# statgen/demuxlet

Measured on AMD Instinct MI355X. Metric: cell-SNP-sample triples/sec (singlet+doublet llk); HBM GB/s vs roofline, higher is better.
Workload: dtype f64

## Files before the change

demuxlet_amd/csrc/dmx_engine.hip:

```cpp
#include <hip/hip_runtime.h>

#include <algorithm>
#include <chrono>
#include <cmath>
#include <mutex>
#include <cstdlib>
#include <cstring>
#include <condition_variable>
#include <deque>
#include <new>
#include <memory>
#include <functional>
#include <thread>
#include <type_traits>
#include <unordered_map>
#include <cxxabi.h>
#include <string>
#include <numeric>
#include <vector>

#include "dmx_internal.hpp"
extern char** environ;
#include "dmx_log.hpp"
#include "dmx_engine_state.hpp"
// ... 3553 lines not shown
#pragma unroll
        for (int i = 0; i < 9; ++i) { P0[i] = P[i]; P1[i] = P[9 + i]; }
        const g_t* gr = &s_g[ti * GS];
        const double a0 = (double)gr[j * 3], a1 = (double)gr[j * 3 + 1], a2 = (double)gr[j * 3 + 2];
        const double aj[3] = {a0, a1, a2};
#pragma unroll
        for (int kk = 0; kk < NK; ++kk) {
          const int k = min(kb * NK + kk, V - 1);
          const double b0 = (double)gr[k * 3], b1 = (double)gr[k * 3 + 1], b2 = (double)gr[k * 3 + 2];
          const double bk[3] = {b0, b1, b2};
          double s0 = (aj[0] * bk[0]) * P0[0], s1 = (aj[0] * bk[0]) * P1[0];
#pragma unroll
          for (int l = 0; l < 3; ++l)
#pragma unroll
            for (int m = 0; m < 3; ++m) {
              if (l == 0 && m == 0) continue;
              const double gp = aj[l] * bk[m];
              s0 += (gp * P0[l * 3 + m]);
              s1 += (gp * P1[l * 3 + m]);
            }
          if (CHK) ok &= __builtin_amdgcn_class(s0, 0x100) && __builtin_amdgcn_class(s1, 0x100);
          acc[kk][0] += dmx_log2_fast_pinned(s0, s_log, lk);
          acc[kk][1] += dmx_log2_fast_pinned(s1, s_log, lk);
        }
      }
    }
    DMX_K2_SYNC();
  }
  if (cell_ok) {
    if constexpr (SYMU) {
#pragma unroll
      for (int su = 0; su < 2; ++su) {
        const int u = tid + TPC * su, d = 1 + (u >> kUSh);
        if (d < kUV / 2 || (d == kUV / 2 && uj[su] < kUV / 2)) {
          double* o = grid + (((size_t)cell * V + uj[su]) * V + uk[su]) * A;
          o[0] = acc[2 * su][0]; o[1] = acc[2 * su][1];
          double* o2 = grid + (((size_t)cell * V + uk[su]) * V + uj[su]) * A;
          o2[0] = acc[2 * su + 1][0]; o2[1] = acc[2 * su + 1][1];
        }
      }
    } else
    if (owner) {
#pragma unroll
      for (int kk = 0; kk < NK; ++kk) {
        const int k = kb * NK + kk;
        if (k < V) {
          double* o = grid + (((size_t)cell * V + j) * V + k) * A;
          o[0] = acc[kk][0]; o[1] = acc[kk][1];
        }
      }
    }
    if (tid < 2 && blockIdx.y == 0) l00[(size_t)cell * A + tid] = acc00;
    if (!ok) flag_cell(flagged, cell);
  }
#undef DMX_K2_SYNC
}
template <int TPC, int NK, int MINW = 1, bool GD = false, bool CHK = true, int TP = 32>
__global__ __launch_bounds__(kThreads, (MINW == 1 && TPC == 64) ? 3 : MINW) void k_doublet_a2(PileupView pv, int nrd_width, const float* __restrict__ g,
                                                         const double* __restrict__ gp0, const double* __restrict__ tabs,
                                                         const double* __restrict__ alpha,
                                                         const int32_t* __restrict__ sched, int32_t V, int32_t GS,
                                                         double* __restrict__ grid, double* __restrict__ l00,
                                                         uint8_t* __restrict__ flagged, const double* __restrict__ pfin, const double* __restrict__ pseed) {
  a2_body<TPC, NK, MINW, GD, CHK, TP, false>(pv, nrd_width, g, gp0, tabs, alpha, sched, V, GS, grid, l00, flagged, pfin, pseed);
}
template <int MINW>
__global__ __launch_bounds__(kThreads, MINW) void k_doublet_a2u(PileupView pv, int nrd_width, const float* __restrict__ g,
                                                          const double* __restrict__ gp0, const double* __restrict__ tabs,
                                                          const double* __restrict__ alpha,
                                                          const int32_t* __restrict__ sched, int32_t V, int32_t GS,
                                                          double* __restrict__ grid, double* __restrict__ l00,
                                                          uint8_t* __restrict__ flagged, const double* __restrict__ pfin, const double* __restrict__ pseed) {
  a2_body<256, 4, MINW, true, false, 32, true>(pv, nrd_width, g, gp0, tabs, alpha, sched, V, GS, grid, l00, flagged, pfin, pseed);
}
__global__ __launch_bounds__(kThreads, 3) void k_doublet_a2u16(PileupView pv, int nrd_width, const float* __restrict__ g,
                                                          const double* __restrict__ gp0, const double* __restrict__ tabs,
                                                          const double* __restrict__ alpha,
                                                          const int32_t* __restrict__ sched, int32_t V, int32_t GS,
                                                          double* __restrict__ grid, double* __restrict__ l00,
                                                          uint8_t* __restrict__ flagged, const double* __restrict__ pfin, const double* __restrict__ pseed) {
  a2_body<64, 4, 1, false, false, 32, true>(pv, nrd_width, g, gp0, tabs, alpha, sched, V, GS, grid, l00, flagged, pfin, pseed);
}

template <int TPC, int NK>
__global__ __launch_bounds__(kThreads, 3) void k_doublet_a2f(PileupView pv, int nrd_width, const float* __restrict__ g,
                                                         const double* __restrict__ gp0, const double* __restrict__ tabs,
                                                         const double* __restrict__ alpha,
                                                         const int32_t* __restrict__ sched, int32_t V, int32_t GS,
                                                         double* __restrict__ grid, double* __restrict__ l00,
                                                         uint8_t* __restrict__ flagged) {
  constexpr int A = 2, TP = 32;
  constexpr int CPW = kThreads / TPC;
  constexpr int T00 = TP + 2;
#define DMX_K2_SYNC() do { if (TPC == 64) { DMX_WAVE_LDS_ORDER(); } else { __syncthreads(); } } while (0)
  extern __shared__ __attribute__((aligned(16))) unsigned char s_raw[];
  __shared__ double s_tab[kTab2];
  const double* s_log = s_tab + kLut2;
  const int t = threadIdx.x;
  stage_k2_tables(s_tab, tabs, t, kThreads);
  __syncthreads();

  const int cw = t / TPC, tid = t % TPC;
  constexpr bool SHARE = TPC > 64;
  constexpr int SUB = 8;
  const int VU = V;
  const size_t cell_bytes = (size_t)TP * 18 * 8 + (size_t)TP * GS * 4 + 2 * T00 * 8 + TP * (4 + 4 + 8) + (SHARE ? (size_t)SUB * 2 * VU * 32 : 0);
  unsigned char* base = s_raw + (size_t)cw * cell_bytes;
  double* s_pG = (double*)base;
  float* s_g = (float*)(base + (size_t)TP * 18 * 8);
  double* s_t00 = (double*)((unsigned char*)s_g + (size_t)TP * GS * 4);
  int64_t* s_off = (int64_t*)(s_t00 + 2 * T00);
  int32_t* s_snp = (int32_t*)(s_off + TP);
  uint32_t* s_cnt = (uint32_t*)(s_snp + TP);
  double* s_u = (double*)(s_cnt + TP);

  const int slot = blockIdx.x * CPW + cw;
  if (TPC == 64 && slot >= pv.B) return;
  const bool cell_ok = slot < pv.B;
  const int32_t cell = cell_ok ? sched[slot] : 0;
  const int64_t p_beg = cell_ok ? pv.cell_pair_off[cell] : 0;
  const int64_t np = cell_ok ? pv.cell_pair_off[cell + 1] - p_beg : 0;
  int64_t rd_base = cell_ok ? pv.cell_read_off[cell] : 0;

  const int KB = (V + NK - 1) / NK;
  const int JS = TPC / KB;
  const int jl = tid / KB, kb = tid % KB;
  const int j = (int)blockIdx.y * JS + jl;
  const bool owner = jl < JS && j < V;
  double acc[NK][A];
#pragma unroll
  for (int kk = 0; kk < NK; ++kk) { acc[kk][0] = 0.0; acc[kk][1] = 0.0; }
  bool ok = true;
  const DmxLogPins lk = dmx_log_pins();
  const int ti1 = tid >> 1, n1 = tid & 1;
  double wA[9], wR[9];
  {
    const double al = alpha[n1];
#pragma unroll
    for (int l = 0; l < 3; ++l)
#pragma unroll
      for (int m = 0; m < 3; ++m) {
        const double p = 0.5 * l + (m - l) * 0.5 * al;
        wA[l * 3 + m] = p;
        wR[l * 3 + m] = 1.0 - p;
      }
  }
  double acc00 = 0.0;
  const int row_len = V * 3;

  for (int64_t tbase = 0; tbase < np; tbase += TP) {
    const int tp = (int)min((int64_t)TP, np - tbase);
    load_tile_headers<TP>(pv, nrd_width, p_beg, tbase, tp, tid, rd_base, s_cnt, s_off, s_snp);
    DMX_K2_SYNC();
    rd_base = s_off[tp - 1] + (int64_t)s_cnt[tp - 1];
    stage_geno_rows<TPC>(g, s_snp, tp, tid, row_len, GS, s_g);
    if (tid < 64) {
      const bool on = ti1 < tp;
      const uint32_t cnt = on ? s_cnt[ti1] : 0u;
      const int64_t off = on ? s_off[ti1] : 0;
      const uint32_t rd4 = load_rd4(pv, off, cnt);
      double pG[9];
      const double mx = pair_values_open<9, 2, true>(pv, cnt, off, rd4, s_tab, wA, wR, n1, pG);
      if (on) {
        const double y = rcp_refined(mx);
        ok &= llks00_term(gp0, s_snp[ti1], [&](int l, int m) { const double v = div_by(pG[l * 3 + m], mx, y); s_pG[(ti1 * 2 + n1) * 9 + l * 3 + m] = v; return v; },
                    s_log, &s_t00[n1 * T00 + ti1]);
// ... 665 lines not shown
#pragma unroll
          for (int c = 0; c < 5; ++c) Pr[c] = pq[c];
#pragma unroll
          for (int c = 0; c < 3; ++c) Qr[c] = pq[5 + c];
        }
        float bn[3] = {gr[kk[0] * 3], gr[kk[0] * 3 + 1], gr[kk[0] * 3 + 2]};
#pragma unroll
        for (int i = 0; i < (DIAG_ONLY ? 0 : NU); ++i) {
          const double b[3] = {(double)bn[0], (double)bn[1], (double)bn[2]};
          if (ROOMY && i + 1 < NU) { const int kn = kk[i + 1]; bn[0] = gr[kn * 3]; bn[1] = gr[kn * 3 + 1]; bn[2] = gr[kn * 3 + 2]; }
          else if (!ROOMY && i + 1 < NU) { const int kn = kk[i + 1]; bn[0] = gr[kn * 3]; bn[1] = gr[kn * 3 + 1]; bn[2] = gr[kn * 3 + 2]; }
          double E[3][3];
#pragma unroll
          for (int l = 0; l < 3; ++l)
#pragma unroll
            for (int m = 0; m < 3; ++m) E[l][m] = a[l] * b[m];
          {
            const double Q[3] = {ROOMY ? Qr[0] : lds_read_f64(&pq[5]), ROOMY ? Qr[1] : lds_read_f64(&pq[6]), ROOMY ? Qr[2] : lds_read_f64(&pq[7])};
            double s_jk0 = E[0][0] * Q[0], s_kj0 = E[0][0] * Q[0];
#pragma unroll
            for (int l = 0; l < 3; ++l)
#pragma unroll
              for (int m = 0; m < 3; ++m) {
                if (l == 0 && m == 0) continue;
                s_jk0 += (E[l][m] * Q[l]);
                s_kj0 += (E[m][l] * Q[l]);
              }
            acc[i][0] += dmx_log2_fast_pinned(s_jk0, s_log, lk);
            acc[i][2] += dmx_log2_fast_pinned(s_kj0, s_log, lk);
          }
          if (!ROOMY) __builtin_amdgcn_sched_barrier(0);
          {
            const double P[5] = {ROOMY ? Pr[0] : lds_read_f64(&pq[0]), ROOMY ? Pr[1] : lds_read_f64(&pq[1]), ROOMY ? Pr[2] : lds_read_f64(&pq[2]),
                                 ROOMY ? Pr[3] : lds_read_f64(&pq[3]), ROOMY ? Pr[4] : lds_read_f64(&pq[4])};
#pragma unroll
            for (int l = 0; l < 3; ++l)
#pragma unroll
              for (int m = 0; m < 3; ++m) E[l][m] = E[l][m] * P[l + m];
            double s_jk1 = E[0][0], s_kj1 = E[0][0];
#pragma unroll
            for (int l = 0; l < 3; ++l)
#pragma unroll
              for (int m = 0; m < 3; ++m) {
                if (l == 0 && m == 0) continue;
                s_jk1 += E[l][m];
                s_kj1 += E[m][l];
              }
            acc[i][1] += dmx_log2_fast_pinned(s_jk1, s_log, lk);
            acc[i][3] += dmx_log2_fast_pinned(s_kj1, s_log, lk);
          }
          __builtin_amdgcn_sched_barrier(0);
        }
        if (slab == 0) {
          double sd = 0.0;
#pragma unroll
          for (int l = 0; l < 3; ++l)
#pragma unroll
            for (int m = 0; m < 3; ++m) {
              const double v = pq[5 + l + dg[m]];
              const double term = (a[l] * a[m]) * v;
              sd = (l == 0 && m == 0) ? term : sd + term;
            }
          accd += dmx_log2_fast_pinned(sd, s_log, lk);
        }
      }
      DMX_WAVE_LDS_ORDER();
    }
  }
  double* G = grid + (size_t)cell * V * V * A;
#pragma unroll
  for (int i = 0; i < (DIAG_ONLY ? 0 : NU); ++i) {
    const int d = 1 + 2 * (NU * slab + i) + h, k = kk[i];
    if (d < 16 || j < 16) {
      G[((size_t)j * V + k) * A] = acc[i][0]; G[((size_t)j * V + k) * A + 1] = acc[i][1];
      G[((size_t)k * V + j) * A] = acc[i][2]; G[((size_t)k * V + j) * A + 1] = acc[i][3];
    }
  }
  if (slab == 0) {
    G[((size_t)j * V + j) * A + h] = accd;
    if (!DIAG_ONLY && tid < 2) l00[(size_t)cell * A + tid] = acc00;
  }
}

template <int MINW, int VP = 32>
__global__ __launch_bounds__(kThreads, MINW) void k_doublet_diag(PileupView pv, int nrd_width, const float* __restrict__ g,
                                                           const double* __restrict__ tabs, const int32_t* __restrict__ sched,
                                                           double* __restrict__ grid, const double* __restrict__ pfin, const double* __restrict__ pseed) {
  static_assert(VP == 32 || VP == 16, "panel");
  constexpr int V = VP, A = 2, TPC = VP, TP = VP / 2, CPW = kThreads / TPC, row_len = 3 * V, PB = 8, WPC = 64 / TPC;
  __shared__ double s_tab[kTab2];
  __shared__ double s_w[2][10];
  __shared__ __attribute__((aligned(16))) double s_pq_all[CPW][TP][8];
  __shared__ int64_t s_off_all[CPW][TP];
  __shared__ int32_t s_snp_all[CPW][TP];
  __shared__ uint32_t s_cnt_all[CPW][TP];
  const double* s_log = s_tab + kLut2;
  const int t = threadIdx.x;
  stage_k2_tables(s_tab, tabs, t, kThreads);
  if (t < 10) {
    const int n = t / 5, q = t % 5;
    const int l = n ? (q > 2 ? 2 : q) : min(q, 2), m = n ? q - l : 0;
    const double p = 0.5 * l + (m - l) * 0.5 * (n ? 0.5 : 0.0);
    s_w[n][q] = p;
    s_w[n][5 + q] = 1.0 - p;
  }
  __syncthreads();
  const int cw = t / TPC, tid = t % TPC;
  double* s_pq = &s_pq_all[cw][0][0];
  int64_t* s_off = s_off_all[cw]; int32_t* s_snp = s_snp_all[cw]; uint32_t* s_cnt = s_cnt_all[cw];
  const int slot = blockIdx.x * CPW + cw;
  if ((blockIdx.x * CPW + (cw & ~(WPC - 1))) >= pv.B) return;
  const bool cell_ok = slot < pv.B;
  const int32_t cell = cell_ok ? sched[slot] : 0;
  const int64_t p_beg = cell_ok ? pv.cell_pair_off[cell] : 0;
  const int64_t np = cell_ok ? pv.cell_pair_off[cell + 1] - p_beg : 0;
  int64_t rd_base = cell_ok ? pv.cell_read_off[cell] : 0;
  int64_t np_w = np;
#pragma unroll
  for (int d = TPC; d < 64; d <<= 1) { const int64_t o = __shfl_xor(np_w, d); np_w = np_w > o ? np_w : o; }
  const int j = tid;
  double acc0 = 0.0, acc1 = 0.0;
  const DmxLogPins lk = dmx_log_pins();
  const int ti1 = tid >> 1, n1 = tid & 1;
  for (int64_t tbase = 0; tbase < np_w; tbase += TP) {
    const int tp = (int)max((int64_t)0, min((int64_t)TP, np - tbase));
    load_tile_headers<TP>(pv, nrd_width, p_beg, tbase, tp, tid, rd_base, s_cnt, s_off, s_snp);
    DMX_WAVE_LDS_ORDER();
    if (tp > 0) rd_base = s_off[tp - 1] + (int64_t)s_cnt[tp - 1];
    {
      const bool on = ti1 < tp;
      const uint32_t cnt = on ? s_cnt[ti1] : 0u;
      const int64_t off = on ? s_off[ti1] : 0;
      const uint32_t rd4 = load_rd4(pv, off, cnt);
      double q[5];
      const int32_t fi = pfin ? certify_final_index(cnt, rd4) : -1;
      if (!__any(fi < 0)) {
        const double* fp = pfin + (size_t)fi * kCFinStride + (n1 ? 0 : 5);
        q[0] = fp[0]; q[1] = fp[1]; q[2] = fp[2];
        q[3] = n1 ? fp[3] : 0.0; q[4] = n1 ? fp[4] : 0.0;
      } else {
        double wA[5], wR[5];
#pragma unroll
        for (int i = 0; i < 5; ++i) { wA[i] = s_w[n1][i]; wR[i] = s_w[n1][5 + i]; }
        certify_pair_values<5, false>(pv, cnt, off, rd4, s_tab, wA, wR, n1, q, pseed);
      }
      if (on) {
        if (n1) {
#pragma unroll
          for (int i = 0; i < 5; ++i) s_pq[ti1 * 8 + i] = q[i];
        } else {
#pragma unroll
          for (int l = 0; l < 3; ++l) s_pq[ti1 * 8 + 5 + l] = q[l];
        }
      }
    }
    DMX_WAVE_LDS_ORDER();
#pragma unroll 1
    for (int sub = 0; sub < TP; sub += PB) {
      if (!__any(sub < tp)) break;
      float ar[PB][3];
#pragma unroll
      for (int pi = 0; pi < PB; ++pi) {
        const float* src = g + (size_t)s_snp[sub + pi] * row_len + j * 3;
        ar[pi][0] = src[0]; ar[pi][1] = src[1]; ar[pi][2] = src[2];
      }
#pragma unroll
      for (int pi = 0; pi < PB; ++pi) {
        if (sub + pi < tp) {
          const double* pq = &s_pq[(sub + pi) * 8];
          const double a[3] = {(double)ar[pi][0], (double)ar[pi][1], (double)ar[pi][2]};
          const double P[5] = {pq[0], pq[1], pq[2], pq[3], pq[4]}, Q[3] = {pq[5], pq[6], pq[7]};
          double s0 = 0.0, s1 = 0.0;
#pragma unroll
          for (int l = 0; l < 3; ++l)
#pragma unroll
            for (int m = 0; m < 3; ++m) {
              const double e = a[l] * a[m];
              const double t0 = e * Q[l], t1 = e * P[l + m];
              s0 = (l == 0 && m == 0) ? t0 : s0 + t0;
              s1 = (l == 0 && m == 0) ? t1 : s1 + t1;
            }
          acc0 += dmx_log2_fast_pinned(s0, s_log, lk);
          acc1 += dmx_log2_fast_pinned(s1, s_log, lk);
        }
      }
    }
    DMX_WAVE_LDS_ORDER();
  }
  if (cell_ok) {
    double* o = grid + (((size_t)cell * V + j) * V + j) * A;
    o[0] = acc0; o[1] = acc1;
  }
}

template <int TPC, int NK, int AP>
__global__ __launch_bounds__(kThreads) void k_doublet_an(PileupView pv, int nrd_width, const float* __restrict__ g,
                                                         const double* __restrict__ gp0, const double* __restrict__ tabs,
                                                         const double* __restrict__ alpha,
                                                         const int32_t* __restrict__ sched, int32_t V, int32_t A, int32_t GS,
                                                         double* __restrict__ grid, double* __restrict__ l00,
                                                         uint8_t* __restrict__ flagged) {
  static_assert(AP == 2 || AP == 4 || AP == 8, "alphas per pair padded to a power of two");
  constexpr int TP = 32;
  constexpr int CPW = kThreads / TPC;
  constexpr int T00 = TP + 2;
#define DMX_K2_SYNC() do { if (TPC == 64) { DMX_WAVE_LDS_ORDER(); } else { __syncthreads(); } } while (0)
  extern __shared__ __attribute__((aligned(16))) unsigned char s_raw[];
  __shared__ double s_tab[kTab2];
  const double* s_log = s_tab + kLut2;
  const int t = threadIdx.x;
  stage_k2_tables(s_tab, tabs, t, kThreads);
  __syncthreads();

  const int cw = t / TPC, tid = t % TPC;
  const size_t cell_bytes = (size_t)TP * AP * 9 * 8 + (size_t)TP * GS * 4 + (size_t)AP * T00 * 8 + TP * (4 + 4 + 8);
  unsigned char* base = s_raw + (size_t)cw * cell_bytes;
  double* s_pG = (double*)base;
  float* s_g = (float*)(base + (size_t)TP * AP * 9 * 8);
  double* s_t00 = (double*)((unsigned char*)s_g + (size_t)TP * GS * 4);
  int64_t* s_off = (int64_t*)(s_t00 + AP * T00);
  int32_t* s_snp = (int32_t*)(s_off + TP);
  uint32_t* s_cnt = (uint32_t*)(s_snp + TP);

  const int slot = blockIdx.x * CPW + cw;
  if (TPC == 64 && slot >= pv.B) return;
  const bool cell_ok = slot < pv.B;
  const int32_t cell = cell_ok ? sched[slot] : 0;
  const int64_t p_beg = cell_ok ? pv.cell_pair_off[cell] : 0;
  const int64_t np = cell_ok ? pv.cell_pair_off[cell + 1] - p_beg : 0;
  int64_t rd_base = cell_ok ? pv.cell_read_off[cell] : 0;

  const int KB = (V + NK - 1) / NK;
  const int JS = TPC / KB;
  const int jl = tid / KB, kb = tid % KB;
  const int j = (int)blockIdx.y * JS + jl;
  const bool owner = jl < JS && j < V;
  double acc[NK][AP];
#pragma unroll
  for (int kk = 0; kk < NK; ++kk)
#pragma unroll
    for (int n = 0; n < AP; ++n) acc[kk][n] = 0.0;
  bool ok = true;
  double acc00 = 0.0;
  const int row_len = V * 3;
  constexpr int P1 = TP * AP;
  constexpr int NPASS = (P1 + TPC - 1) / TPC;
  const int n1 = tid % AP;
  const bool n_ok = n1 < A;
  double wA[9], wR[9];
  {
    const double al = n_ok ? alpha[n1] : 0.0;
#pragma unroll
    for (int l = 0; l < 3; ++l)
#pragma unroll
      for (int m = 0; m < 3; ++m) {
        const double p = 0.5 * l + (m - l) * 0.5 * al;
        wA[l * 3 + m] = p;
        wR[l * 3 + m] = 1.0 - p;
      }
  }

  for (int64_t tbase = 0; tbase < np; tbase += TP) {
    const int tp = (int)min((int64_t)TP, np - tbase);
    load_tile_headers<TP>(pv, nrd_width, p_beg, tbase, tp, tid, rd_base, s_cnt, s_off, s_snp);
    DMX_K2_SYNC();
    rd_base = s_off[tp - 1] + (int64_t)s_cnt[tp - 1];
    stage_geno_rows<TPC>(g, s_snp, tp, tid, row_len, GS, s_g);
#pragma unroll
    for (int pass = 0; pass < NPASS; ++pass) {
      const int u = tid + pass * TPC;
      if (u >= P1) break;
      const int ti1 = u / AP;
      const bool on = ti1 < tp && n_ok;
      const uint32_t cnt = (ti1 < tp) ? s_cnt[ti1] : 0u;
      const int64_t off = (ti1 < tp) ? s_off[ti1] : 0;
// ... 3044 lines not shown
    DMX_LAUNCH(k2_fn, (k_doublet_sym<TPC, VMAX, SUB, FIX>), dim3((unsigned)((B + (kThreads / TPC) - 1) / (kThreads / TPC))), \
                       block, lds, e->stream, e->pv, e->nrd_width, e->d_g, e->d_gp0, e->d_lut, e->d_sched, V | sym_flags,           \
                       e->d_grid, e->d_l00, e->d_flag(), pfin, pseed);                                                                \
  } while (0)
#define DMX_K2SV(TPC, VMAX, SUB, FIX, MINW)                                                                            \
  do { e->k2_sym = true;                                                                                                                \
    constexpr int GSS_ = (3 * VMAX + 3) & ~3, VUS_ = (VMAX + 2) & ~1, TP_ = TPC >= 64 ? 32 : TPC / 2;                   \
    constexpr size_t cb_ = (size_t)TP_ * 6 * 8 + TP_ * 4 * 8 + 2 * (TP_ + 2) * 8 + TP_ * 16 + (size_t)(TPC == 32 ? 3 : (TPC >= 32 ? 2 : 1)) * SUB * GSS_ * 4 + (size_t)SUB * 3 * VUS_ * 8; \
    const size_t lds = cb_ * (kThreads / TPC);                                                                         \
    if (lds > 60 * 1024) HIP_TRY(hipFuncSetAttribute(reinterpret_cast<const void*>(&k_doublet_sym<TPC, VMAX, SUB, FIX, MINW>), \
                                                     hipFuncAttributeMaxDynamicSharedMemorySize, (int)lds));          \
    DMX_LAUNCH(k2_fn, (k_doublet_sym<TPC, VMAX, SUB, FIX, MINW>), dim3((unsigned)((B + (kThreads / TPC) - 1) / (kThreads / TPC))), \
                       block, lds, e->stream, e->pv, e->nrd_width, e->d_g, e->d_gp0, e->d_lut, e->d_sched, V | sym_flags,           \
                       e->d_grid, e->d_l00, e->d_flag(), pfin, pseed);                                                                \
  } while (0)
    const int32_t sym_flags = (e->knob("DMX_SYM_NO_DMA") ? (1 << 16) : 0) | (e->knob("DMX_SYM_ABLATE_P1") ? (1 << 17) : 0) |
                              (e->knob("DMX_SYM_ABLATE_P2") ? (1 << 18) : 0) | (e->knob("DMX_SYM_ABLATE_U") ? (1 << 19) : 0) |
                              (e->knob("DMX_SYM_ABLATE_RD") ? (1 << 20) : 0) | (e->knob("DMX_SYM_ABLATE_00") ? (1 << 21) : 0) | (e->knob("DMX_SYM_NO_PRODUCT") ? (1 << 22) : 0) |
                              (e->knob("DMX_SYM_NO_PIPE") ? (1 << 23) : 0) | (e->knob("DMX_SYM_WAIT_ALL") ? (1 << 24) : 0);
    const bool wide_cells = e->knob("DMX_SYM_ONE_CELL_PER_WAVE") != nullptr;
    if (V <= 8 && !wide_cells) { if (16 % V == 0) DMX_K2S(16, 8, 4, true); else DMX_K2S(16, 8, 4, false); }
    else if (V <= 16 && !wide_cells) { if (V == 16) DMX_K2S(32, 16, 4, true); else DMX_K2S(32, 16, 4, false); }
    else if (V <= 8) { if (64 % V == 0) DMX_K2S(64, 8, 4, true); else DMX_K2S(64, 8, 4, false); }
    else if (V <= 17) { if (V == 16) DMX_K2S(64, 17, 4, true); else DMX_K2S(64, 17, 4, false); }
    else if (V <= 23) DMX_K2S(64, 23, 4, false);
    else if (V <= 27) DMX_K2S(64, 27, 4, false);
    else if (V <= 32) {
      if (V == 32) {
        const int var = e->knob("DMX_SYM_VARIANT") ? atoi(e->knob("DMX_SYM_VARIANT")) : 0;
        if (var == 1) DMX_K2SV(64, 32, 2, true, 4); else if (var == 2) DMX_K2SV(64, 32, 4, true, 4); else if (var == 3) DMX_K2SV(64, 32, 8, true, 3);
        else if (var == 4) DMX_K2SV(64, 32, 2, true, 3); else if (var == 5) DMX_K2SV(64, 32, 8, true, 2); else DMX_K2S(64, 32, 4, true);
      } else DMX_K2S(64, 32, 4, false);
    }
    else if (V <= 48) DMX_K2S(256, 48, 8, false);
    else if (V <= 64) { if (V == 64) DMX_K2S(256, 64, 8, true); else DMX_K2S(256, 64, 8, false); }
    else {
      const unsigned ns = (unsigned)((V * (V / 2 + 1) + V + 256 * 9 - 1) / (256 * 9));
#define DMX_K2SS(VMAX, SUB, FIX)                                                                                       \
  do { e->k2_sym = true;                                                                                                                \
    constexpr int GSS_ = (3 * VMAX + 3) & ~3, VUS_ = (VMAX + 2) & ~1;                                                  \
    constexpr size_t cb_ = (size_t)32 * 6 * 8 + 32 * 4 * 8 + 2 * 34 * 8 + 32 * 16 + (size_t)2 * SUB * GSS_ * 4 + (size_t)SUB * 3 * VUS_ * 8; \
    HIP_TRY(hipFuncSetAttribute(reinterpret_cast<const void*>(&k_doublet_sym<256, VMAX, SUB, FIX, 3, 9>),              \
                                hipFuncAttributeMaxDynamicSharedMemorySize, (int)cb_));                               \
    HIP_TRY(hipFuncSetAttribute(reinterpret_cast<const void*>(&k_doublet_sym<256, VMAX, SUB, FIX, 3, 9, false>),       \
                                hipFuncAttributeMaxDynamicSharedMemorySize, (int)cb_));                               \
    if (e->geno_safe)                                                                                                  \
      DMX_LAUNCH(k2_fn, (k_doublet_sym<256, VMAX, SUB, FIX, 3, 9, false>), dim3((unsigned)B, ns), block, cb_, e->stream, e->pv, \
                         e->nrd_width, e->d_g, e->d_gp0, e->d_lut, e->d_sched, V | sym_flags, e->d_grid, e->d_l00, e->d_flag(), pfin, pseed);      \
    else                                                                                                               \
    DMX_LAUNCH(k2_fn, (k_doublet_sym<256, VMAX, SUB, FIX, 3, 9>), dim3((unsigned)B, ns), block, cb_, e->stream, e->pv, \
                       e->nrd_width, e->d_g, e->d_gp0, e->d_lut, e->d_sched, V | sym_flags, e->d_grid, e->d_l00, e->d_flag(), pfin, pseed);        \
  } while (0)
      if (V <= 96) DMX_K2SS(96, 8, false); else if (V == 128) DMX_K2SS(128, 8, true); else if (V < 128) DMX_K2SS(128, 8, false);
      else if (V <= 192) DMX_K2SS(192, 4, false); else if (V <= 256) DMX_K2SS(256, 4, false);
      else if (V <= 384) DMX_K2SS(384, 2, false); else DMX_K2SS(512, 2, false);
#undef DMX_K2SS
    }
#undef DMX_K2SV
#undef DMX_K2S
    HIP_TRY(hipGetLastError());
    return launch_doublet_generic_w<true>(e);
  }
  if (fast_soft && V <= 128) {
    const size_t fast_bytes = cell_bytes + (V > 16 ? (size_t)8 * 2 * V * 32 : 0);
#define DMX_K2F(TPC, NK)                                                                                             \
  do {                                                                                                               \
    const size_t lds = fast_bytes * (kThreads / TPC);                                                                \
    if (lds > 60 * 1024) HIP_TRY(hipFuncSetAttribute(reinterpret_cast<const void*>(&k_doublet_a2f<TPC, NK>),          \
                                                     hipFuncAttributeMaxDynamicSharedMemorySize, (int)lds));          \
    DMX_LAUNCH(k2_fn, (k_doublet_a2f<TPC, NK>), dim3((unsigned)((B + (kThreads / TPC) - 1) / (kThreads / TPC)), slabs_of(TPC, NK)), \
                       block, lds, e->stream, e->pv, e->nrd_width, e->d_g, e->d_gp0, e->d_lut, e->d_alpha, e->d_sched, V, GS,           \
                       e->d_grid, e->d_l00, e->d_flag());                                                              \
  } while (0)
    if (V <= 8) DMX_K2F(64, 1);
    else if (V <= 16) DMX_K2F(64, 4);
    else if (V <= 32) DMX_K2F(256, 4);
    else DMX_K2F(256, 16);
#undef DMX_K2F
    HIP_TRY(hipGetLastError());
    return launch_doublet_generic_w<true>(e);
  }
  if (V == 32 && pfin_a2_grid && e->geno_safe && !e->knob("DMX_A2_SYM") && !e->knob("DMX_A2_NO_SYMU") && !e->knob("DMX_A2_NO_GD") && !e->knob("DMX_A2_MINW1")) {
    const size_t cbd = (size_t)32 * 18 * 8 + (size_t)32 * GS * 8 + 2 * 34 * 8 + 32 * (4 + 4 + 8);
    DMX_LAUNCH(k2_fn, (k_doublet_a2u<4>), dim3((unsigned)B, 1), block, cbd, e->stream, e->pv, e->nrd_width, e->d_g,
                       e->d_gp0, e->d_lut, e->d_alpha, e->d_sched, V, GS, e->d_grid, e->d_l00, e->d_flag(), pfin_a2, pseed_a2);
    if (e->knob("DMX_A2U_DIAG_WAVE"))
      hipLaunchKernelGGL((k_doublet_a2s<4, 4, 0>), dim3((unsigned)((B + 3) / 4), 1), block, 0, e->stream, e->pv, e->nrd_width, e->d_g, e->d_gp0, e->d_lut, e->d_sched,
                         e->d_grid, e->d_l00, pfin_a2);
    else
      hipLaunchKernelGGL((k_doublet_diag<5>), dim3((unsigned)((B + 7) / 8)), block, 0, e->stream, e->pv, e->nrd_width, e->d_g, e->d_lut, e->d_sched, e->d_grid, pfin_a2, pseed_a2);
  }
  else if (V == 32 && pfin_a2_grid && e->geno_safe && e->knob("DMX_A2_SYM")) {
    const dim3 grds((unsigned)((B + 3) / 4), 2);
    if (e->knob("DMX_A2S_SUB8"))
      DMX_LAUNCH(k2_fn, (k_doublet_a2s<8, 3>), grds, block, 0, e->stream, e->pv, e->nrd_width, e->d_g, e->d_gp0, e->d_lut, e->d_sched, e->d_grid, e->d_l00, pfin_a2);
    else if (!e->knob("DMX_A2S_MINW4"))
      DMX_LAUNCH(k2_fn, (k_doublet_a2s<4, 3>), grds, block, 0, e->stream, e->pv, e->nrd_width, e->d_g, e->d_gp0, e->d_lut, e->d_sched, e->d_grid, e->d_l00, pfin_a2);
    else
      DMX_LAUNCH(k2_fn, (k_doublet_a2s<4, 4>), grds, block, 0, e->stream, e->pv, e->nrd_width, e->d_g, e->d_gp0, e->d_lut, e->d_sched, e->d_grid, e->d_l00, pfin_a2);
  }
  else if (V == 16 && pfin_a2_grid && e->geno_safe && !e->knob("DMX_A2_NO_SYMU")) {
    DMX_LAUNCH(k2_fn, (k_doublet_a2u16), dim3((unsigned)((B + 3) / 4), 1), block, cell_bytes * 4, e->stream, e->pv, e->nrd_width, e->d_g,
                       e->d_gp0, e->d_lut, e->d_alpha, e->d_sched, V, GS, e->d_grid, e->d_l00, e->d_flag(), pfin_a2, pseed_a2);
    hipLaunchKernelGGL((k_doublet_diag<5, 16>), dim3((unsigned)((B + 15) / 16)), block, 0, e->stream, e->pv, e->nrd_width, e->d_g, e->d_lut, e->d_sched, e->d_grid, pfin_a2, pseed_a2);
  }
  else if (V <= 8) DMX_K2A(64, 1);
  else if (V <= 16) DMX_K2A(64, 4);
  else if (V <= 32) {
    if (!e->knob("DMX_A2_NO_GD") && !e->knob("DMX_A2_MINW1")) {
      const size_t cbd = (size_t)32 * 18 * 8 + (size_t)32 * GS * 8 + 2 * 34 * 8 + 32 * (4 + 4 + 8);
      if (e->geno_safe)
        DMX_LAUNCH(k2_fn, (k_doublet_a2<256, 4, 4, true, false>), dim3((unsigned)B, slabs_of(256, 4)), block, cbd, e->stream, e->pv, e->nrd_width, e->d_g,
                           e->d_gp0, e->d_lut, e->d_alpha, e->d_sched, V, GS, e->d_grid, e->d_l00, e->d_flag(), pfin_a2, pseed_a2);
      else
      DMX_LAUNCH(k2_fn, (k_doublet_a2<256, 4, 4, true>), dim3((unsigned)B, slabs_of(256, 4)), block, cbd, e->stream, e->pv, e->nrd_width, e->d_g,
                         e->d_gp0, e->d_lut, e->d_alpha, e->d_sched, V, GS, e->d_grid, e->d_l00, e->d_flag(), pfin_a2, pseed_a2);
    } else if (!e->knob("DMX_A2_MINW1"))
      DMX_LAUNCH(k2_fn, (k_doublet_a2<256, 4, 4>), dim3((unsigned)B, slabs_of(256, 4)), block, cell_bytes, e->stream, e->pv, e->nrd_width, e->d_g,
                         e->d_gp0, e->d_lut, e->d_alpha, e->d_sched, V, GS, e->d_grid, e->d_l00, e->d_flag(), pfin_a2, pseed_a2);
    else DMX_K2A(256, 4);
  }
  else if (V <= 128) DMX_K2A(256, 16);
  else {
    auto bytes_of = [&](int tp) { return (size_t)tp * 18 * 8 + (size_t)tp * GS * 4 + 2 * (size_t)(tp + 2) * 8 + (size_t)tp * (4 + 4 + 8); };
    constexpr size_t kStatic = sizeof(double) * kTab2 + 2 * 18 * sizeof(double), kTwo = 80 * 1024, kOne = 160 * 1024;
    int tp = 0;
    for (int c : {32, 16, 8}) if (!tp && bytes_of(c) + kStatic <= kTwo) tp = c;
    for (int c : {32, 16, 8}) if (!tp && bytes_of(c) + kStatic <= kOne) tp = c;
    if (const char* env = e->knob("DMX_A2_TP")) { const int c = atoi(env); if ((c == 32 || c == 16 || c == 8) && bytes_of(c) + kStatic <= kOne) tp = c; }
    if (!tp) return set_error(DMX_ERR_ARG, "run_doublet: V = %d exceeds k_doublet_a2's LDS budget", (int)V);
    const size_t lds = bytes_of(tp);
#define DMX_K2AW(TPP)                                                                                                 \
  do {                                                                                                                \
    if (e->geno_safe) {                                                                                               \
      if (lds > 60 * 1024) HIP_TRY(hipFuncSetAttribute(reinterpret_cast<const void*>(&k_doublet_a2<256, 16, 1, false, false, TPP>),  \
                                                       hipFuncAttributeMaxDynamicSharedMemorySize, (int)lds));        \
      DMX_LAUNCH(k2_fn, (k_doublet_a2<256, 16, 1, false, false, TPP>), dim3((unsigned)B, slabs_of(256, 16)), block, lds, e->stream, e->pv,  \
                         e->nrd_width, e->d_g, e->d_gp0, e->d_lut, e->d_alpha, e->d_sched, V, GS, e->d_grid, e->d_l00, e->d_flag(), pfin_a2, pseed_a2);  \
    } else {                                                                                                          \
      if (lds > 60 * 1024) HIP_TRY(hipFuncSetAttribute(reinterpret_cast<const void*>(&k_doublet_a2<256, 16, 1, false, true, TPP>),   \
                                                       hipFuncAttributeMaxDynamicSharedMemorySize, (int)lds));        \
      DMX_LAUNCH(k2_fn, (k_doublet_a2<256, 16, 1, false, true, TPP>), dim3((unsigned)B, slabs_of(256, 16)), block, lds, e->stream, e->pv,   \
                         e->nrd_width, e->d_g, e->d_gp0, e->d_lut, e->d_alpha, e->d_sched, V, GS, e->d_grid, e->d_l00, e->d_flag(), pfin_a2, pseed_a2);  \
    }                                                                                                                 \
  } while (0)
    if (tp == 32) DMX_K2AW(32); else if (tp == 16) DMX_K2AW(16); else DMX_K2AW(8);
#undef DMX_K2AW
  }
#undef DMX_K2A
  HIP_TRY(hipGetLastError());
  return launch_doublet_generic_w<true>(e);
}

}

namespace {
int launch_certify(dmx_engine* e) {
  const int32_t B = e->pv.B;
  const int64_t* blk = (e->pv.pair_snp && e->blk_n > 1 && (e->knob("DMX_CERTIFY_BLOCKS") || e->knob("DMX_K1_BLOCK_BYTES"))) ? e->d_blk : nullptr;
  const int bstride = (blk && e->knob("DMX_CERTIFY_BLOCK_STRIDE")) ? std::max(1, atoi(e->knob("DMX_CERTIFY_BLOCK_STRIDE"))) : 1;
  const int n_launch = blk ? (e->blk_n + bstride - 1) / bstride : 1;
  double* park = nullptr;
  if (blk) {
    if (int rc = e->d_park.ensure(sizeof(double) * kPark * (size_t)std::max(B, 1))) return rc;
    park = e->d_park;
  }
  const float* gT = (!e->pv.pair_snp && e->have_gT && !e->knob("DMX_CERTIFY_NO_GT")) ? e->d_gT : nullptr;
#define DMX_K3B(MINW_, FIVE_, DENSE_)                                                                                  \
  for (int bi = 0; bi < n_launch; ++bi)                                                                                 \
// ... 2585 lines not shown
```

Measured before the change: 14.61 billion.

## Add two-cell-per-block symmetric doublet kernel for V=32 with split diagonal work

Adds a new V=32 doublet grid kernel that processes two cells per block, sharing the staged genotype rows. It splits the upper-triangle pair work across two y-slabs, with each thread computing the jk and kj entries for both cells. Log2 lookups are software-pipelined with explicit waitcnt and sched barriers. Half of the diagonal is folded into the main kernel, and a new 16-lane diagonal kernel handles the rest. This is meant to raise reuse and occupancy, at the cost of more code complexity and of assuming that both cells share one SNP schedule.

```diff
diff --git a/demuxlet_amd/csrc/dmx_engine.hip b/demuxlet_amd/csrc/dmx_engine.hip
--- a/demuxlet_amd/csrc/dmx_engine.hip
+++ b/demuxlet_amd/csrc/dmx_engine.hip
@@ -3659,6 +3659,231 @@
   a2_body<64, 4, 1, false, false, 32, true>(pv, nrd_width, g, gp0, tabs, alpha, sched, V, GS, grid, l00, flagged, pfin, pseed);
 }
 
+struct k_doublet_a2u2 { static constexpr bool diag16 = true; };
+struct k_doublet_a2u2_whole_diag_behind { static constexpr bool diag16 = false; };
+template <bool DIAG16>
+__device__ __forceinline__ void a2u2_body(PileupView pv, int nrd_width, const float* __restrict__ g,
+                                                         const double* __restrict__ gp0, const double* __restrict__ tabs,
+                                                         const double* __restrict__ alpha, const int32_t* __restrict__ sched,
+                                                         double* __restrict__ grid, double* __restrict__ l00,
+                                                         uint8_t* __restrict__ flagged, const double* __restrict__ pfin, const double* __restrict__ pseed) {
+  constexpr int V = 32, A = 2, TP = 32, T00 = TP + 2, GS = 3 * V, row_len = 3 * V;
+  __shared__ double s_tab[kTab2];
+  __shared__ double s_w[2][18];
+  __shared__ __attribute__((aligned(16))) double s_q[2][TP][8];
+  __shared__ __attribute__((aligned(16))) double s_g[TP * GS];
+  __shared__ __attribute__((aligned(16))) double s_t00[2][2][T00];
+  __shared__ int64_t s_off[2][TP];
+  __shared__ int32_t s_snp[2][TP];
+  __shared__ uint32_t s_cnt[2][TP];
+  const double* s_log = s_tab + kLut2;
+  const int tid = threadIdx.x;
+  stage_k2_tables(s_tab, tabs, tid, kThreads);
+  if (tid < 18) {
+    const int n = tid / 9, l = (tid % 9) / 3, m = tid % 3;
+    const double p = 0.5 * l + (m - l) * 0.5 * alpha[n];
+    s_w[n][tid % 9] = p;
+    s_w[n][9 + tid % 9] = 1.0 - p;
+  }
+  __syncthreads();
+
+  const int slot0 = 2 * (int)blockIdx.x;
+  const bool two = slot0 + 1 < pv.B;
+  const bool slab0 = blockIdx.y == 0;
+  const int hb = (tid >> 5) & 1, hl = tid & 31;
+  const int bb = (tid >> 6) & 1, ti1 = (tid & 63) >> 1, n1 = tid & 1;
+  const int32_t cell0 = sched[slot0], cell1 = two ? sched[slot0 + 1] : cell0;
+  const int32_t cell_h = hb ? cell1 : cell0;
+  const int64_t p_beg = pv.cell_pair_off[cell_h];
+  int64_t rd_base = pv.cell_read_off[cell_h];
+  const int np = (int)(pv.cell_pair_off[cell0 + 1] - pv.cell_pair_off[cell0]);
+
+  const int u = tid + kThreads * (int)blockIdx.y, uj = u & 31, ud = 1 + (u >> 5);
+  const bool udiag = DIAG16 && u >= 496;
+  const int uk = udiag ? uj : (uj + ud) & 31;
+  const double* const ga = s_g + uj * 3;
+  const double* const gb = s_g + uk * 3;
+  double acc[2][4];
+#pragma unroll
+  for (int c = 0; c < 2; ++c) { acc[c][0] = 0.0; acc[c][1] = 0.0; acc[c][2] = 0.0; acc[c][3] = 0.0; }
+  bool ok = true;
+  double acc00 = 0.0;
+  const DmxLogPins lk = dmx_log_pins();
+
+  for (int tbase = 0; tbase < np; tbase += TP) {
+    const int tp = min(TP, np - tbase);
+    if (tid < 64) load_tile_headers<TP>(pv, nrd_width, p_beg, (int64_t)tbase, tp, hl, rd_base, s_cnt[hb], s_off[hb], s_snp[hb]);
+    __syncthreads();
+    if (tid < 64) rd_base = s_off[hb][tp - 1] + (int64_t)s_cnt[hb][tp - 1];
+    stage_geno_rows<kThreads>(g, s_snp[0], tp, tid, row_len, GS, s_g);
+    if (tid < 4 * TP) {
+      const bool on = ti1 < tp;
+      const uint32_t cnt = on ? s_cnt[bb][ti1] : 0u;
+      const int64_t off = on ? s_off[bb][ti1] : 0;
+      const uint32_t rd4 = load_rd4(pv, off, cnt);
+      double vf[9];
+      const int32_t fi = pfin ? certify_final_index(cnt, rd4) : -1;
+      if (!__any(fi < 0)) {
+        const double* fp = pfin + (size_t)fi * kCFinStride + (n1 ? 0 : 5);
+        const double f0 = fp[0], f1 = fp[1], f2 = fp[2], f3 = n1 ? fp[3] : 0.0, f4 = n1 ? fp[4] : 0.0;
+        const double f5[5] = {f0, f1, f2, f3, f4};
+#pragma unroll
+        for (int l = 0; l < 3; ++l)
+#pragma unroll
+          for (int m = 0; m < 3; ++m) vf[l * 3 + m] = n1 ? f5[l + m] : f5[l];
+      } else if (pseed) {
+        double q5[5], wA5[5], wR5[5];
+#pragma unroll
+        for (int q = 0; q < 5; ++q) {
+          const int l = n1 ? (q > 2 ? 2 : q) : min(q, 2), m = n1 ? q - l : 0;
+          const double p = 0.5 * l + (m - l) * 0.5 * (n1 ? 0.5 : 0.0);
+          wA5[q] = p;
+          wR5[q] = 1.0 - p;
+        }
+        certify_pair_values<5, false>(pv, cnt, off, rd4, s_tab, wA5, wR5, n1, q5, pseed);
+#pragma unroll
+        for (int l = 0; l < 3; ++l)
+#pragma unroll
+          for (int m = 0; m < 3; ++m) vf[l * 3 + m] = n1 ? q5[l + m] : q5[l];
+      } else {
+        double wA[9], wR[9];
+#pragma unroll
+        for (int i = 0; i < 9; ++i) { wA[i] = s_w[n1][i]; wR[i] = s_w[n1][9 + i]; }
+        certify_pair_values<9, false, 2, true>(pv, cnt, off, rd4, s_tab, wA, wR, n1, vf);
+      }
+      if (on) {
+        double* q = &s_q[bb][ti1][0];
+        if (n1) { q[0] = vf[0]; q[1] = vf[1]; q[2] = vf[2]; q[3] = vf[5]; q[4] = vf[8]; }
+        else { q[5] = vf[0]; q[6] = vf[3]; q[7] = vf[6]; }
+        if (slab0)
+          ok &= llks00_term(gp0, s_snp[bb][ti1], [&](int l, int m) { return vf[l * 3 + m]; }, s_log, &s_t00[bb][n1][ti1]);
+      }
+    }
+    __syncthreads();
+    if (slab0 && tid < 4) {
+      const double* row = &s_t00[tid >> 1][tid & 1][0];
+      if (tp == TP) {
+        double2 v[TP / 2];
+#pragma unroll
+        for (int i = 0; i < TP / 2; ++i) v[i] = *reinterpret_cast<const double2*>(&row[2 * i]);
+#pragma unroll
+        for (int i = 0; i < TP / 2; ++i) { acc00 += v[i].x; acc00 += v[i].y; }
+      } else {
+        for (int i = 0; i < tp; ++i) acc00 += row[i];
+      }
+    }
+    {
+      const int tps = __builtin_amdgcn_readfirstlane(tp);
+      double Q[2][3], P1[2][5], ar[3], br[3];
+      auto load_pair = [&](int pi) {
+#pragma unroll
+        for (int c = 0; c < 2; ++c) {
+          const double* q = &s_q[c][pi][0];
+          P1[c][0] = q[0]; P1[c][1] = q[1]; P1[c][2] = q[2]; P1[c][3] = q[3]; P1[c][4] = q[4];
+          Q[c][0] = q[5]; Q[c][1] = q[6]; Q[c][2] = q[7];
+        }
+        const double* ra = &ga[pi * GS];
+        const double* rb = &gb[pi * GS];
+        ar[0] = ra[0]; ar[1] = ra[1]; ar[2] = ra[2];
+        br[0] = rb[0]; br[1] = rb[1]; br[2] = rb[2];
+      };
+      load_pair(0);
+      for (int ti = 0; ti < tps; ++ti) {
+        double E[3][3], T1[3][3];
+#pragma unroll
+        for (int l = 0; l < 3; ++l)
+#pragma unroll
+          for (int m = 0; m < 3; ++m) E[l][m] = ar[l] * br[m];
+        double s_jk0[2], s_kj0[2], s_jk1[2], s_kj1[2];
+#pragma unroll
+        for (int c = 0; c < 2; ++c) {
+          s_jk0[c] = E[0][0] * Q[c][0]; s_kj0[c] = E[0][0] * Q[c][0];
+#pragma unroll
+          for (int l = 0; l < 3; ++l)
+#pragma unroll
+            for (int m = 0; m < 3; ++m) {
+              if (l == 0 && m == 0) continue;
+              s_jk0[c] += (E[l][m] * Q[c][l]);
+              s_kj0[c] += (E[m][l] * Q[c][l]);
+            }
+        }
+#pragma unroll
+        for (int l = 0; l < 3; ++l)
+#pragma unroll
+          for (int m = 0; m < 3; ++m) {
+            T1[l][m] = E[l][m] * P1[1][l + m];
+            E[l][m] = E[l][m] * P1[0][l + m];
+          }
+        s_jk1[0] = E[0][0]; s_kj1[0] = E[0][0];
+#pragma unroll
+        for (int l = 0; l < 3; ++l)
+#pragma unroll
+          for (int m = 0; m < 3; ++m) {
+            if (l == 0 && m == 0) continue;
+            s_jk1[0] += E[l][m];
+            s_kj1[0] += E[m][l];
+          }
+        const DmxLog2Req a_jk0 = dmx_log2_request_fast(s_jk0[0], s_log), a_kj0 = dmx_log2_request_fast(s_kj0[0], s_log),
+                         a_jk1 = dmx_log2_request_fast(s_jk1[0], s_log), a_kj1 = dmx_log2_request_fast(s_kj1[0], s_log);
+        __builtin_amdgcn_sched_barrier(0);
+        s_jk1[1] = T1[0][0]; s_kj1[1] = T1[0][0];
+#pragma unroll
+        for (int l = 0; l < 3; ++l)
+#pragma unroll
+          for (int m = 0; m < 3; ++m) {
+            if (l == 0 && m == 0) continue;
+            s_jk1[1] += T1[l][m];
+            s_kj1[1] += T1[m][l];
+          }
+        __builtin_amdgcn_sched_barrier(0);
+        __builtin_amdgcn_s_waitcnt(0xC07F);
+        __builtin_amdgcn_sched_barrier(0);
+        const DmxLog2Req b_jk0 = dmx_log2_request_fast(s_jk0[1], s_log), b_kj0 = dmx_log2_request_fast(s_kj0[1], s_log),
+                         b_jk1 = dmx_log2_request_fast(s_jk1[1], s_log), b_kj1 = dmx_log2_request_fast(s_kj1[1], s_log);
+        load_pair(min(ti + 1, tps - 1));
+        __builtin_amdgcn_sched_barrier(0);
+        acc[0][0] += dmx_log2_finish_pinned(a_jk0, lk);
+        acc[0][1] += dmx_log2_finish_pinned(a_kj0, lk);
+        acc[0][2] += dmx_log2_finish_pinned(a_jk1, lk);
+        acc[0][3] += dmx_log2_finish_pinned(a_kj1, lk);
+        asm volatile("" : "+v"(acc[0][0]), "+v"(acc[0][1]), "+v"(acc[0][2]), "+v"(acc[0][3]));
+        __builtin_amdgcn_sched_barrier(0);
+        __builtin_amdgcn_s_waitcnt(0xC07F);
+        __builtin_amdgcn_sched_barrier(0);
+        acc[1][0] += dmx_log2_finish_pinned(b_jk0, lk);
+        acc[1][1] += dmx_log2_finish_pinned(b_kj0, lk);
+        acc[1][2] += dmx_log2_finish_pinned(b_jk1, lk);
+        acc[1][3] += dmx_log2_finish_pinned(b_kj1, lk);
+        __builtin_amdgcn_sched_barrier(0);
+      }
+    }
+    __syncthreads();
+  }
+  if (ud < 16 || (ud == 16 && uj < 16) || udiag) {
+#pragma unroll
+    for (int c = 0; c < 2; ++c) {
+      if (c == 1 && !two) break;
+      const int32_t cell = c ? cell1 : cell0;
+      double* o = grid + (((size_t)cell * V + uj) * V + uk) * A;
+      o[0] = acc[c][0]; o[1] = acc[c][2];
+      if (!udiag) {
+        double* o2 = grid + (((size_t)cell * V + uk) * V + uj) * A;
+        o2[0] = acc[c][1]; o2[1] = acc[c][3];
+      }
+    }
+  }
+  if (slab0 && tid < 4 && (tid < 2 || two)) l00[(size_t)((tid >> 1) ? cell1 : cell0) * A + (tid & 1)] = acc00;
+  if (!ok) flag_cell(flagged, bb ? cell1 : cell0);
+}
+template <class FORM>
+__global__ __launch_bounds__(kThreads, 4) void k_doublet_a2u(PileupView pv, int nrd_width, const float* __restrict__ g,
+                                                         const double* __restrict__ gp0, const double* __restrict__ tabs,
+                                                         const double* __restrict__ alpha, const int32_t* __restrict__ sched,
+                                                         double* __restrict__ grid, double* __restrict__ l00,
+                                                         uint8_t* __restrict__ flagged, const double* __restrict__ pfin, const double* __restrict__ pseed) {
+  a2u2_body<FORM::diag16>(pv, nrd_width, g, gp0, tabs, alpha, sched, grid, l00, flagged, pfin, pseed);
+}
+
 template <int TPC, int NK>
 __global__ __launch_bounds__(kThreads, 3) void k_doublet_a2f(PileupView pv, int nrd_width, const float* __restrict__ g,
                                                          const double* __restrict__ gp0, const double* __restrict__ tabs,
@@ -4490,12 +4715,12 @@
   }
 }
 
-template <int MINW, int VP = 32>
-__global__ __launch_bounds__(kThreads, MINW) void k_doublet_diag(PileupView pv, int nrd_width, const float* __restrict__ g,
+template <int MINW, int VP, int LN>
+__device__ __forceinline__ void diag_body(PileupView pv, int nrd_width, const float* __restrict__ g,
                                                            const double* __restrict__ tabs, const int32_t* __restrict__ sched,
                                                            double* __restrict__ grid, const double* __restrict__ pfin, const double* __restrict__ pseed) {
-  static_assert(VP == 32 || VP == 16, "panel");
-  constexpr int V = VP, A = 2, TPC = VP, TP = VP / 2, CPW = kThreads / TPC, row_len = 3 * V, PB = 8, WPC = 64 / TPC;
+  static_assert((VP == 32 || VP == 16) && (LN == VP || LN == 16), "panel");
+  constexpr int V = VP, A = 2, TPC = LN, TP = LN / 2, CPW = kThreads / TPC, row_len = 3 * V, PB = 8, WPC = 64 / TPC;
   __shared__ double s_tab[kTab2];
   __shared__ double s_w[2][10];
   __shared__ __attribute__((aligned(16))) double s_pq_all[CPW][TP][8];
@@ -4599,6 +4824,18 @@
     double* o = grid + (((size_t)cell * V + j) * V + j) * A;
     o[0] = acc0; o[1] = acc1;
   }
+}
+template <int MINW, int VP = 32>
+__global__ __launch_bounds__(kThreads, MINW) void k_doublet_diag(PileupView pv, int nrd_width, const float* __restrict__ g,
+                                                           const double* __restrict__ tabs, const int32_t* __restrict__ sched,
+                                                           double* __restrict__ grid, const double* __restrict__ pfin, const double* __restrict__ pseed) {
+  diag_body<MINW, VP, VP>(pv, nrd_width, g, tabs, sched, grid, pfin, pseed);
+}
+template <int MINW>
+__global__ __launch_bounds__(kThreads, MINW) void k_doublet_diag_lo(PileupView pv, int nrd_width, const float* __restrict__ g,
+                                                           const double* __restrict__ tabs, const int32_t* __restrict__ sched,
+                                                           double* __restrict__ grid, const double* __restrict__ pfin, const double* __restrict__ pseed) {
+  diag_body<MINW, 32, 16>(pv, nrd_width, g, tabs, sched, grid, pfin, pseed);
 }
 
 template <int TPC, int NK, int AP>
@@ -7809,9 +8046,20 @@
   }
   if (V == 32 && pfin_a2_grid && e->geno_safe && !e->knob("DMX_A2_SYM") && !e->knob("DMX_A2_NO_SYMU") && !e->knob("DMX_A2_NO_GD") && !e->knob("DMX_A2_MINW1")) {
     const size_t cbd = (size_t)32 * 18 * 8 + (size_t)32 * GS * 8 + 2 * 34 * 8 + 32 * (4 + 4 + 8);
+    const bool two_barcodes = e->pv.pair_snp == nullptr && !e->knob("DMX_A2U_ONE_BARCODE");
+    const bool diag16 = two_barcodes && !e->knob("DMX_A2U2_NO_DIAG") && !e->knob("DMX_A2U_DIAG_WAVE");
+    if (diag16)
+      DMX_LAUNCH(k2_fn, (k_doublet_a2u<k_doublet_a2u2>), dim3((unsigned)((B + 1) / 2), 2), block, 0, e->stream, e->pv, e->nrd_width, e->d_g,
+                         e->d_gp0, e->d_lut, e->d_alpha, e->d_sched, e->d_grid, e->d_l00, e->d_flag(), pfin_a2, pseed_a2);
+    else if (two_barcodes)
+      DMX_LAUNCH(k2_fn, (k_doublet_a2u<k_doublet_a2u2_whole_diag_behind>), dim3((unsigned)((B + 1) / 2), 2), block, 0, e->stream, e->pv, e->nrd_width, e->d_g,
+                         e->d_gp0, e->d_lut, e->d_alpha, e->d_sched, e->d_grid, e->d_l00, e->d_flag(), pfin_a2, pseed_a2);
+    else
     DMX_LAUNCH(k2_fn, (k_doublet_a2u<4>), dim3((unsigned)B, 1), block, cbd, e->stream, e->pv, e->nrd_width, e->d_g,
                        e->d_gp0, e->d_lut, e->d_alpha, e->d_sched, V, GS, e->d_grid, e->d_l00, e->d_flag(), pfin_a2, pseed_a2);
-    if (e->knob("DMX_A2U_DIAG_WAVE"))
+    if (diag16)
+      hipLaunchKernelGGL((k_doublet_diag_lo<5>), dim3((unsigned)((B + 15) / 16)), block, 0, e->stream, e->pv, e->nrd_width, e->d_g, e->d_lut, e->d_sched, e->d_grid, pfin_a2, pseed_a2);
+    else if (e->knob("DMX_A2U_DIAG_WAVE"))
       hipLaunchKernelGGL((k_doublet_a2s<4, 4, 0>), dim3((unsigned)((B + 3) / 4), 1), block, 0, e->stream, e->pv, e->nrd_width, e->d_g, e->d_gp0, e->d_lut, e->d_sched,
                          e->d_grid, e->d_l00, pfin_a2);
     else
```

Measured after the change: 15.22 billion, median of 6. +4.2%, better.
